# g-ch/DSP-map

Measured on AMD Instinct MI355X. Metric: map update() frames/sec @ 66x66x40, 24 particles/voxel; achieved HBM GB/s, higher is better.
Workload: dtype f32; 1 GPU; B: 66x66x40 @ 0.15 m, 24 particles/voxel, synthetic 640x480 depth @ 30 Hz (corridor scene, <=5000 points/frame after 0.1 m voxel filter), steady state after 300 frames; parallelism=1 GPU, n_points=3706, storage=runs of 64 voxel indices

## Files before the change

dsp-map_amd/csrc/dspmap_birth.h:

```cpp
#pragma once
#include "dspmap_device.h"

template <int NB>
__device__ __forceinline__ int block_excl_scan_multi(int (&v)[NB], int* s_tmp) {
    const int tid = threadIdx.x, w = tid >> 6, l = tid & 63, nw = blockDim.x >> 6;
    int inc[NB];
#pragma unroll
    for (int j = 0; j < NB; ++j) {
        inc[j] = wave_incl_scan_i(v[j]);
        if (l == 63) s_tmp[j * 16 + w] = inc[j];
    }
    __syncthreads();
    if (w == 0) {
        int run = 0;
#pragma unroll
        for (int j = 0; j < NB; ++j) {
            const int t = l < nw ? s_tmp[j * 16 + l] : 0;
            const int ti = wave_incl_scan_i(t);
            if (l < nw) s_tmp[j * 16 + l] = run + ti - t;
            run += __builtin_amdgcn_readlane(ti, 63);
        }
        if (l == 0) s_tmp[NB * 16] = run;
    }
    __syncthreads();
#pragma unroll
    for (int j = 0; j < NB; ++j) v[j] = inc[j] - v[j] + s_tmp[j * 16 + w];
    const int total = s_tmp[NB * 16];
    __syncthreads();
    return total;
}


#define BK 8
struct BirthView {
    const BirthSrc* stored;
    const float4* rot;
    const int* pyr;
    float cx, cy, cz;
    int n;
    bool live;
};
__device__ __forceinline__ BirthView birth_view(const DevState& s) {
    BirthView v;
    const FrameParams* fp = s.fpar;
    const int mode = fp->static_birth;
    v.live = mode == 1 && s.fs->view_epoch == fp->epoch;
    v.stored = fp->birth; v.rot = s.pt_rot; v.pyr = s.pt_pyr;
    v.cx = fp->cur_pos[0]; v.cy = fp->cur_pos[1]; v.cz = fp->cur_pos[2];
    v.n = mode == 1 ? (v.live ? fp->n_pts : s.fs->stale_n) : (mode == 2 ? s.fs->est_n : fp->n_birth);
    return v;
}
__device__ __forceinline__ BirthSrc birth_at(const BirthView& v, int i) {
    if (!v.live) return v.stored[i];
    const float4 r = v.rot[i];
    BirthSrc b;
    b.x = r.x + v.cx; b.y = r.y + v.cy; b.z = r.z + v.cz;
    b.nx = b.ny = b.nz = 0.f;
    b.intensity = v.pyr[i] >= 0 ? 0.f : -2.f;
    return b;
}
__device__ __forceinline__ bool birth_src_voxel(const MapDims& d, const DevState& s, const BirthSrc& src, float& cx, float& cy, float& cz, int& gv,
                                                const float* cp = nullptr) {
    if (!cp) cp = s.fs->cur_pos;
    cx = src.x - cp[0];
    cy = src.y - cp[1];
    cz = src.z - cp[2];
    if (!(src.intensity > -1.5f)) return false;
    if (voxel_of(d, cx, cy, cz, gv)) return true;
    gv = 0;
    return d.static_model != 0;
}

__device__ __forceinline__ void birth_rank_block(const MapDims& d, const DevState& s, const FilterParams& fp, bool fpar_pos = false) {
    const BirthView bv = birth_view(s);
    const float* cp = fpar_pos ? s.fpar->cur_pos : nullptr;
    const int n_birth = bv.n;
    __shared__ int s_tmp[BK * 16 + 1];
    const int tid = threadIdx.x, nt = blockDim.x;
    const int p_cur = s.fs->p_cur;
    const int nb = fp.nb_num;
    int run = 0;
    for (int base = 0; base < n_birth; base += nt * BK) {
        int v[BK];
        bool ok[BK];
#pragma unroll
        for (int j = 0; j < BK; ++j) {
            const int i = base + j * nt + tid;
            float cx, cy, cz; int gv;
            ok[j] = i < n_birth && birth_src_voxel(d, s, birth_at(bv, i), cx, cy, cz, gv, cp);
            v[j] = ok[j] ? 1 : 0;
            if (i < n_birth) s.plan_inside[i] = 0u;
        }
        const int tot = block_excl_scan_multi<BK>(v, s_tmp);
#pragma unroll
        for (int j = 0; j < BK; ++j)
            if (ok[j]) s.plan_pbase[base + j * nt + tid] = (int)(((long long)p_cur + 3ll * nb * (long long)(run + v[j])) % fp.tab_n);
        run += tot;
    }
    if (tid == 0) { s.fs->p_cur = (int)(((long long)p_cur + 3ll * nb * run) % fp.tab_n); s.fs->n_birth_ovf = 0; }
}

#define BIRTH_BUCKET_CAP 128
__device__ __forceinline__ void birth_child_thread(const MapDims& d, const DevState& s, const FilterParams& fp, float4* __restrict__ child,
                                                   int* __restrict__ vb_cnt, int* __restrict__ vb_idx, const int t, bool* inside_out = nullptr) {
    const BirthView bv = birth_view(s);
    const int n_birth = bv.n;
    const int nb = fp.nb_num;
    const int i = t / nb, k = t - i * nb;
    if (i >= n_birth) return;
    float cx, cy, cz; int gsrc;
    if (!birth_src_voxel(d, s, birth_at(bv, i), cx, cy, cz, gsrc)) return;
    const int c = (int)(((long long)s.plan_pbase[i] + 3 * k) % fp.tab_n);
    const float x = cx + s.p_tab[c];
    const float y = cy + s.p_tab[(c + 1) % fp.tab_n];
    const float z = cz + s.p_tab[(c + 2) % fp.tab_n];
    int gv = 0;
    int lv = -1;
    if (voxel_of_lv(d, x, y, z, gv, lv)) {
        if (inside_out) *inside_out = true; else atomicOr(&s.plan_inside[i], 1u << k);
        if (lv >= 0) {
            const int pos = atomicAdd(&vb_cnt[lv], 1);
            if (pos < BIRTH_BUCKET_CAP) vb_idx[(size_t)lv * BIRTH_BUCKET_CAP + pos] = t;
            else s.birth_ovf[atomicAdd(&s.fs->n_birth_ovf, 1)] = t;
        } else {
            lv = -1;
        }
    }
    child[t] = make_float4(x, y, z, __int_as_float(lv));
}
```

dsp-map_amd/csrc/dspmap_device.h:

```cpp
#pragma once
#include <hip/hip_runtime.h>
#include "dspmap_types.h"

#define WAVE 64

__device__ __forceinline__ int lane_id() { return (int)__lane_id(); }
__device__ __forceinline__ int sload_i(const int* p) {
    int v;
    asm volatile("s_load_dword %0, %1, 0x0\n\ts_waitcnt lgkmcnt(0)" : "=s"(v) : "s"(p));
    return v;
}
__device__ __forceinline__ void sload_i3(const int* p0, const int* p1, const int* p2, int& v0, int& v1, int& v2) {
    asm volatile("s_load_dword %0, %3, 0x0\n\ts_load_dword %1, %4, 0x0\n\ts_load_dword %2, %5, 0x0\n\ts_waitcnt lgkmcnt(0)"
                 : "=&s"(v0), "=&s"(v1), "=&s"(v2) : "s"(p0), "s"(p1), "s"(p2));
}
__device__ __forceinline__ void sload_i5(const int* p0, const int* p1, const int* p2, const int* p3, const int* p4, int& v0, int& v1, int& v2, int& v3, int& v4) {
    asm volatile("s_load_dword %0, %5, 0x0\n\ts_load_dword %1, %6, 0x0\n\ts_load_dword %2, %7, 0x0\n\ts_load_dword %3, %8, 0x0\n\ts_load_dword %4, %9, 0x0\n\ts_waitcnt lgkmcnt(0)"
                 : "=&s"(v0), "=&s"(v1), "=&s"(v2), "=&s"(v3), "=&s"(v4) : "s"(p0), "s"(p1), "s"(p2), "s"(p3), "s"(p4));
}
__device__ __forceinline__ void sload_i2(const int* p0, const int* p1, int& v0, int& v1) {
    asm volatile("s_load_dword %0, %2, 0x0\n\ts_load_dword %1, %3, 0x0\n\ts_waitcnt lgkmcnt(0)" : "=&s"(v0), "=&s"(v1) : "s"(p0), "s"(p1));
}
__device__ __forceinline__ void sload_i4(const int* p0, const int* p1, const int* p2, const int* p3, int& v0, int& v1, int& v2, int& v3) {
    asm volatile("s_load_dword %0, %4, 0x0\n\ts_load_dword %1, %5, 0x0\n\ts_load_dword %2, %6, 0x0\n\ts_load_dword %3, %7, 0x0\n\ts_waitcnt lgkmcnt(0)"
                 : "=&s"(v0), "=&s"(v1), "=&s"(v2), "=&s"(v3) : "s"(p0), "s"(p1), "s"(p2), "s"(p3));
}
__device__ __forceinline__ u64 lanemask_lt() { return (1ull << lane_id()) - 1ull; }

template <int CTRL, int ROW_MASK>
__device__ __forceinline__ float dpp_add_f(float v) {
    return v + __int_as_float(__builtin_amdgcn_update_dpp(0, __float_as_int(v), CTRL, ROW_MASK, 0xf, false));
}
template <int CTRL, int ROW_MASK>
__device__ __forceinline__ int dpp_add_i(int v) {
    return v + __builtin_amdgcn_update_dpp(0, v, CTRL, ROW_MASK, 0xf, false);
}
__device__ __forceinline__ float wave_incl_scan(float v) {
    v = dpp_add_f<0x111, 0xf>(v);
    v = dpp_add_f<0x112, 0xf>(v);
    v = dpp_add_f<0x114, 0xf>(v);
    v = dpp_add_f<0x118, 0xf>(v);
    v = dpp_add_f<0x142, 0xa>(v);
    v = dpp_add_f<0x143, 0xc>(v);
    return v;
}
__device__ __forceinline__ int wave_incl_scan_i(int v) {
    v = dpp_add_i<0x111, 0xf>(v);
    v = dpp_add_i<0x112, 0xf>(v);
    v = dpp_add_i<0x114, 0xf>(v);
    v = dpp_add_i<0x118, 0xf>(v);
    v = dpp_add_i<0x142, 0xa>(v);
    v = dpp_add_i<0x143, 0xc>(v);
    return v;
}
__device__ __forceinline__ float wave_sum(float v) {
    return __int_as_float(__builtin_amdgcn_readlane(__float_as_int(wave_incl_scan(v)), 63));
}
__device__ __forceinline__ float wave_sum_f(float v) {
#pragma unroll
    for (int o = 32; o > 0; o >>= 1) v += __shfl_xor(v, o, WAVE);
    return v;
}
__device__ __forceinline__ int wave_sum_i(int v) { return __builtin_amdgcn_readlane(wave_incl_scan_i(v), 63); }

__device__ __forceinline__ int wave_agg_inc(int* cnt, int key, bool active) {
    int pos = -1;
    u64 todo = __ballot(active);
    const int l = lane_id();
    while (todo) {
        const int leader = __ffsll((long long)todo) - 1;
        const int k = __shfl(key, leader, WAVE);
        const bool mine = active && key == k;
        const u64 grp = __ballot(mine);
        int base = 0;
        if (l == leader) base = atomicAdd(&cnt[k], (int)__popcll(grp));
        base = __shfl(base, leader, WAVE);
        if (mine) pos = base + (int)__popcll(grp & ((1ull << l) - 1ull));
        todo &= ~grp;
    }
    return pos;
}
__device__ __forceinline__ int wave_agg_inc1(int* cnt, bool active) {
    const u64 grp = __ballot(active);
    if (!grp) return -1;
    const int l = lane_id();
    const int leader = __ffsll((long long)grp) - 1;
    int base = 0;
    if (l == leader) base = atomicAdd(cnt, (int)__popcll(grp));
    base = __shfl(base, leader, WAVE);
    return active ? base + (int)__popcll(grp & ((1ull << l) - 1ull)) : -1;
}
__device__ __forceinline__ void wave_count_add(int* cnt, bool active) {
    const u64 grp = __ballot(active);
    if (grp && lane_id() == __ffsll((long long)grp) - 1) atomicAdd(cnt, (int)__popcll(grp));
}

__device__ __forceinline__ unsigned wave_or_u32(unsigned v) {
    v |= (unsigned)__builtin_amdgcn_update_dpp(0, (int)v, 0x111, 0xf, 0xf, false);
    v |= (unsigned)__builtin_amdgcn_update_dpp(0, (int)v, 0x112, 0xf, 0xf, false);
    v |= (unsigned)__builtin_amdgcn_update_dpp(0, (int)v, 0x114, 0xf, 0xf, false);
    v |= (unsigned)__builtin_amdgcn_update_dpp(0, (int)v, 0x118, 0xf, 0xf, false);
    v |= (unsigned)__builtin_amdgcn_update_dpp(0, (int)v, 0x142, 0xa, 0xf, false);
    v |= (unsigned)__builtin_amdgcn_update_dpp(0, (int)v, 0x143, 0xc, 0xf, false);
    return (unsigned)__builtin_amdgcn_readlane((int)v, 63);
}
__device__ __forceinline__ u64 wave_or_u64(u64 v) {
    return ((u64)wave_or_u32((unsigned)(v >> 32)) << 32) | (u64)wave_or_u32((unsigned)v);
}
__device__ __forceinline__ void quat_mul(const float a[4], const float b[4], float r[4]) {
    r[0] = a[0] * b[0] - a[1] * b[1] - a[2] * b[2] - a[3] * b[3];
    r[1] = a[0] * b[1] + a[1] * b[0] + a[2] * b[3] - a[3] * b[2];
    r[2] = a[0] * b[2] + a[2] * b[0] + a[3] * b[1] - a[1] * b[3];
    r[3] = a[0] * b[3] + a[3] * b[0] + a[1] * b[2] - a[2] * b[1];
}
__device__ __forceinline__ void rotate_by_quat(float vx, float vy, float vz, const float q[4], float out[3]) {
    float vq[4] = {0.f, vx, vy, vz};
    float n2 = q[1] * q[1] + q[2] * q[2] + q[3] * q[3] + q[0] * q[0];
    float inv[4] = {__fdiv_rn(q[0], n2), __fdiv_rn(-q[1], n2), __fdiv_rn(-q[2], n2), __fdiv_rn(-q[3], n2)};
    float t[4], r[4];
    quat_mul(q, vq, t);
    quat_mul(t, inv, r);
    out[0] = r[1]; out[1] = r[2]; out[2] = r[3];
}

__device__ __forceinline__ float dot3(float x, float y, float z, const float* n) {
    return x * n[0] + y * n[1] + z * n[2];
}

__device__ __forceinline__ int pyramid_of(const MapDims& d, const float* ph, const float* pv, float x, float y, float z) {
    if (!(dot3(x, y, z, ph) >= 0.f && dot3(x, y, z, ph + 3 * d.np_h) <= 0.f &&
          dot3(x, y, z, pv) <= 0.f && dot3(x, y, z, pv + 3 * d.np_v) >= 0.f))
        return -1;
    int lo = 0, hi = d.np_h - 1;
    while (lo < hi) {
        int mid = (lo + hi) >> 1;
        if (dot3(x, y, z, ph + 3 * (mid + 1)) <= 0.f) hi = mid; else lo = mid + 1;
    }
    const int h = lo;
    lo = 0; hi = d.np_v - 1;
    while (lo < hi) {
        int mid = (lo + hi) >> 1;
        if (dot3(x, y, z, pv + 3 * (mid + 1)) >= 0.f) hi = mid; else lo = mid + 1;
    }
    return h * d.np_v + lo;
}

__device__ __forceinline__ float div_res(const MapDims& d, float a) {
    if (d.div_ok) {
        const float q0 = a * d.rcp_res;
        const float r = __fmaf_rn(-q0, d.res, a);
        return __fmaf_rn(r, d.rcp_res, q0);
    }
    return __fdiv_rn(a, d.res);
}
__device__ __forceinline__ bool voxel_of(const MapDims& d, float px, float py, float pz, int& gidx) {
    if (fabsf(px) >= d.half_x || fabsf(py) >= d.half_y || fabsf(pz) >= d.half_z) return false;
    const int x = (int)div_res(d, px + d.half_x);
    const int y = (int)div_res(d, py + d.half_y);
    const int z = (int)div_res(d, pz + d.half_z);
    gidx = (int)(__umul24((unsigned)z, (unsigned)(d.ny * d.nx)) + __umul24((unsigned)y, (unsigned)d.nx) + (unsigned)x);
    return (unsigned)gidx < (unsigned)d.v_glob;
}

__device__ __forceinline__ int lv_of_xyz(const MapDims& d, int x, int y, int zl) {
    if (!d.tiling) return (int)(__umul24((unsigned)zl, (unsigned)(d.ny * d.nx)) + __umul24((unsigned)y, (unsigned)d.nx) + (unsigned)x);
    return ((((zl >> 2) * d.ncy + (y >> 2)) * d.ncx + (x >> 2)) << 6) | ((zl & 3) << 4) | ((y & 3) << 2) | (x & 3);
}
__device__ __forceinline__ int lv_of_true(const MapDims& d, int t) {
    if (!d.tiling) return t;
    const int zc = d.ny * d.nx;
    const int zl = t / zc, rest = t - zl * zc, y = rest / d.nx, x = rest - y * d.nx;
    return lv_of_xyz(d, x, y, zl);
}
__device__ __forceinline__ int lv_of_g(const MapDims& d, int gv) {
    const int t = gv - d.v_base;
    return (t >= 0 && t < d.v_true) ? lv_of_true(d, t) : -1;
}
__device__ __forceinline__ int g_of_lv(const MapDims& d, int lv) {
    if (!d.tiling) return lv + d.v_base;
    const int c = lv >> 6;
    const int cx = c % d.ncx, r = c / d.ncx, cy = r % d.ncy, cz = r / d.ncy;
    const int x = cx * 4 + (lv & 3), y = cy * 4 + ((lv >> 2) & 3), zl = cz * 4 + ((lv >> 4) & 3);
    if (x >= d.nx || y >= d.ny || zl >= d.z_hi - d.z_lo) return -1;
    return ((d.z_lo + zl) * d.ny + y) * d.nx + x;
}
__device__ __forceinline__ int tile_gbase(const MapDims& d, int BX) {
    if (!d.tiling) return d.v_base + BX * 64;
    const int cx = BX % d.ncx, r = BX / d.ncx, cy = r % d.ncy, cz = r / d.ncy;
    return ((d.z_lo + cz * 4) * d.ny + cy * 4) * d.nx + cx * 4;
}
__device__ __forceinline__ int lane_goff(const MapDims& d, int lane) {
    return d.tiling ? (((lane >> 4) & 3) * d.ny + ((lane >> 2) & 3)) * d.nx + (lane & 3) : lane;
}
__device__ __forceinline__ void cube_box(const MapDims& d, int BX, int& x0, int& y0, int& z0) {
    const int cx = BX % d.ncx, r = BX / d.ncx, cy = r % d.ncy, cz = r / d.ncy;
    x0 = cx * 4; y0 = cy * 4; z0 = d.z_lo + cz * 4;
}
__device__ __forceinline__ bool voxel_of_lv(const MapDims& d, float px, float py, float pz, int& gidx, int& lv) {
    if (fabsf(px) >= d.half_x || fabsf(py) >= d.half_y || fabsf(pz) >= d.half_z) return false;
    const int x = (int)div_res(d, px + d.half_x);
    const int y = (int)div_res(d, py + d.half_y);
    const int z = (int)div_res(d, pz + d.half_z);
    gidx = (int)(__umul24((unsigned)z, (unsigned)(d.ny * d.nx)) + __umul24((unsigned)y, (unsigned)d.nx) + (unsigned)x);
    if (!((unsigned)gidx < (unsigned)d.v_glob)) return false;
    const int zl = z - d.z_lo;
    lv = (unsigned)zl < (unsigned)(d.z_hi - d.z_lo) ? lv_of_xyz(d, x, y, zl) : -1;
    return true;
}

__device__ __forceinline__ float axis_u(float a, float mu, float sigma, float inv_sigma) {
    const float dlt = a - mu;
    const float q0 = dlt * inv_sigma;
    const float rr = __fmaf_rn(-q0, sigma, dlt);
    float z = __fmaf_rn(rr, inv_sigma, q0);
    z = __builtin_amdgcn_fmed3f(z, -9.9f, 9.9f);
    return floorf(z * 1000.f + 10000.f) - 10000.f;
}
__device__ __forceinline__ float pair_gk(float px, float py, float pz, float ox, float oy, float oz,
                                         float sigma, float inv_sigma, float c3) {
    const float ux = axis_u(px, ox, sigma, inv_sigma);
    const float uy = axis_u(py, oy, sigma, inv_sigma);
    const float uz = axis_u(pz, oz, sigma, inv_sigma);
    const float s = ux * ux + uy * uy + uz * uz;
    return c3 * __builtin_amdgcn_exp2f(s * -7.213475204444817e-07f);
}

typedef float f2v __attribute__((ext_vector_type(2)));
__device__ __forceinline__ f2v axis_u2(f2v a, f2v mu, float sigma, float inv_sigma) {
    const f2v dlt = a - mu;
    const f2v q0 = dlt * inv_sigma;
    const f2v rr = __builtin_elementwise_fma(-q0, (f2v)(sigma), dlt);
    f2v z = __builtin_elementwise_fma(rr, (f2v)(inv_sigma), q0);
    z.x = __builtin_amdgcn_fmed3f(z.x, -9.9f, 9.9f);
// ... 182 lines not shown
```

dsp-map_amd/csrc/dspmap_kernels.hip:

```cpp
#include <hip/hip_runtime.h>
#include "dspmap_device.h"
#include "dspmap_kernels.h"
#include "dspmap_birth.h"

#define RESET_PLANES 1
#define RESET_OBS 2
#define RESET_PRED 4

__global__ void k_reset(MapDims d, DevState s, int flags) {
    const float qw = s.fpar->quat[0], qx = s.fpar->quat[1], qy = s.fpar->quat[2], qz = s.fpar->quat[3];
    const float cx = s.fpar->cur_pos[0], cy = s.fpar->cur_pos[1], cz = s.fpar->cur_pos[2];
    const int gt = blockIdx.x * blockDim.x + threadIdx.x;
    const int gn = gridDim.x * blockDim.x;
    if (flags & RESET_PLANES) {
        const float q[4] = {qw, qx, qy, qz};
        const int nh = d.np_h + 1, nv = d.np_v + 1;
        for (int i = gt; i < nh + nv; i += gn) {
            float o[3];
            if (i < nh) {
                rotate_by_quat(s.planes_h0[3 * i], s.planes_h0[3 * i + 1], s.planes_h0[3 * i + 2], q, o);
                s.planes_h[3 * i] = o[0]; s.planes_h[3 * i + 1] = o[1]; s.planes_h[3 * i + 2] = o[2];
            } else {
                const int j = i - nh;
                rotate_by_quat(s.planes_v0[3 * j], s.planes_v0[3 * j + 1], s.planes_v0[3 * j + 2], q, o);
// ... 793 lines not shown
            const int wave = tid >> 6, l = tid & 63;
            const u64 cmask = (spl == 1 ? ~0ull : spl == 2 ? 0x5555555555555555ull : spl == 4 ? 0x1111111111111111ull : 0x0101010101010101ull) << sub;
            int run = 0, round = 0;
            for (int base = 0; base < O; base += WU_TPB, ++round) {
                const int o = base + tid;
                bool keep = false;
                float4 z = make_float4(0.f, 0.f, 0.f, 0.f);
                int oi = 0;
                if (o < O) {
                    int k = 0;
                    for (int q = 1; q < d.nbins; ++q) k += (o >= s_off[q]) ? 1 : 0;
                    oi = s_bin[k] * DSP_OBS_CAP + (o - s_off[k]);
                    z = s.obs[oi];
                    keep = z.w >= lo && z.w <= hi;
                }
                const u64 bal = __ballot(keep) & cmask;
                int* wc = s_wc + (round & 1) * 32;
                if (l < spl) wc[wave * 8 + l] = (int)__popcll(bal);
                __syncthreads();
                int off = run, tot = 0;
                for (int w = 0; w < WU_TPB / 64; ++w) { const int c = wc[w * 8 + sub]; tot += c; off += w < wave ? c : 0; }
                if (keep) {
                    const int pos = (off + (int)__popcll(bal & lanemask_lt())) * spl + sub;
                    s_len[pos] = z.w;
                    z.w = __fdiv_rn(fp.p_det, ck_from_fix(s.obs_ck[oi]) + add);
                    s_o[pos] = z;
                }
                run += tot;
            }
            n_mine = run;
        }
        __syncthreads();
        float sum = 0.f;
        if (valid && !occluded) {
            if (SKIP) {
                for (int j = 0; j < n_mine; ++j) {
                    const int o = j * spl + sub;
                    if (fabsf(s_len[o] - dist) > fp.cull_r) continue;
                    const float4 z = s_o[o];
                    sum += pair_gk(p.x, p.y, p.z, z.x, z.y, z.z, fp.sigma_ob, fp.inv_sigma_ob, fp.pdf_c3) * z.w;
                }
            } else {
                int o = sub;
                for (; o + spl < O; o += 2 * spl) {
                    const float4 z = s_o[o], z2 = s_o[o + spl];
                    const f2v gk = pair_gk2(f2v{p.x, p.x}, f2v{p.y, p.y}, f2v{p.z, p.z}, f2v{z.x, z2.x}, f2v{z.y, z2.y}, f2v{z.z, z2.z},
                                            fp.sigma_ob, fp.inv_sigma_ob, fp.pdf_c3);
                    if (fabsf(s_len[o] - dist) <= fp.cull_r) sum += gk.x * z.w;
                    if (fabsf(s_len[o + spl] - dist) <= fp.cull_r) sum += gk.y * z2.w;
                }
                if (o < O && fabsf(s_len[o] - dist) <= fp.cull_r) {
                    const float4 z = s_o[o];
                    sum += pair_gk(p.x, p.y, p.z, z.x, z.y, z.z, fp.sigma_ob, fp.inv_sigma_ob, fp.pdf_c3) * z.w;
                }
            }
        }
        if (spl >= 2) sum += __shfl_xor(sum, 1, WAVE);
        if (spl >= 4) sum += __shfl_xor(sum, 2, WAVE);
        if (spl >= 8) sum += __shfl_xor(sum, 4, WAVE);
        if (valid && !occluded && sub == 0) s.w[s.fov_slot_s[ri]] = p.w * ((1.f - fp.p_det) + sum);
    }
}

__device__ __forceinline__ void birth_split_wave(const MapDims& d, const DevState& s, const FilterParams& fp, int i, int2* cvr = nullptr,
                                                 const unsigned* inside_in = nullptr) {
    const BirthView bv = birth_view(s);
    if (cvr) *cvr = make_int2(0, 0);
    if (i >= bv.n) return;
    const int l = lane_id();
    const BirthSrc src = birth_at(bv, i);
    BirthPlan pl;
    pl.gvox = -1; pl.n_static = 0; pl.inside = 0; pl.pbase = pl.vbase = pl.rbase = 0;
    int gv;
    const bool ok = birth_src_voxel(d, s, src, pl.cx, pl.cy, pl.cz, gv);
    int n_static = 0;
    if (ok) {
        pl.gvox = gv;
        const int lv = lv_of_g(d, gv);
        if (lv >= 0) {
            float ws = 0.f, wsd = 0.f, wd = 0.f;
            for (int e = 0; e < d.mw; ++e) {
                const int sl = e * 64 + l;
                const u64 m = s.mask[(size_t)lv * d.mw + e] & ~s.nbmask[(size_t)lv * d.mw + e];
                if (sl < d.slots && ((m >> l) & 1ull)) {
                    const size_t idx = pidx(d, lv, sl);
                    const V2 pv = ld_vel(s, idx);
                    const float vabs = fabsf(pv.x) + fabsf(pv.y) + 0.f;
                    const float w = s.w[idx];
                    if (vabs < 0.1f) ws += w; else if (vabs < 0.5f) wsd += w; else wd += w;
                }
            }
            ws = wave_sum(ws); wsd = wave_sum(wsd); wd = wave_sum(wd);
            const float total = ws + wd + wsd;
            const float m_s = __fdiv_rn(ws, total), m_d = __fdiv_rn(wd, total), m_sd = __fdiv_rn(wsd, total);
            const float p_s = (m_s + m_s + m_sd) * 0.5f;
            const float p_d = (m_d + m_d + m_sd) * 0.5f;
            const float p_s_n = __fdiv_rn(p_s, p_s + p_d);
            const float f = (float)fp.model_nb * p_s_n;
            int ns = (f != f) ? 0 : (int)f;
            n_static = max(fp.min_static_nb, ns);
        }
    }
    pl.n_static = n_static;
    if (l == 0) { s.plan[i] = pl; s.nstatic[i] = n_static; }
    if (cvr && ok && src.intensity > 0.01f) {
        const unsigned inside = inside_in ? *inside_in : s.plan_inside[i];
        const int nb = fp.nb_num;
        const int model_end = src.nx > -100.f ? fp.model_nb : n_static;
        auto below = [](int k) { return k >= 32 ? ~0u : ((1u << k) - 1u); };
        const int lo = min(n_static, nb), mid = min(max(model_end, lo), nb);
        *cvr = make_int2(3 * __popc(inside & below(mid) & ~below(lo)), 3 * __popc(inside & below(nb) & ~below(mid)));
    }
}
__global__ void k_birth_split(MapDims d, DevState s, FilterParams fp) {
    birth_split_wave(d, s, fp, (int)(blockIdx.x * (blockDim.x / WAVE) + threadIdx.x / WAVE));
}

__device__ __forceinline__ void birth_point_wave(const MapDims& d, const DevState& s, const FilterParams& fp, int i, float4* __restrict__ child,
                                                 int* __restrict__ vb_cnt, int* __restrict__ vb_idx, int2* cvr) {
    const BirthView bv = birth_view(s);
    *cvr = make_int2(0, 0);
    if (i >= bv.n) return;
    const int l = lane_id(), nb = fp.nb_num;
    const BirthSrc src = birth_at(bv, i);
    const int pb = s.plan_pbase[i];
    BirthPlan pl;
    pl.gvox = -1; pl.n_static = 0; pl.inside = 0; pl.pbase = pl.vbase = pl.rbase = 0;
    int gv;
    const bool ok = birth_src_voxel(d, s, src, pl.cx, pl.cy, pl.cz, gv);
    if (!ok) {
        if (l == 0) { s.plan[i] = pl; s.nstatic[i] = 0; s.plan_inside[i] = 0u; }
        return;
    }
    pl.gvox = gv;
    const int lvs = lv_of_g(d, gv);
    const bool own = lvs >= 0;
    const int lvq = own ? lvs : 0;
    const int c = (int)(((long long)pb + 3 * min(l, nb - 1)) % fp.tab_n);
    const float t0 = s.p_tab[c], t1 = s.p_tab[(c + 1) % fp.tab_n], t2 = s.p_tab[(c + 2) % fp.tab_n];
    u64 mwd[2] = {0ull, 0ull};
    for (int e = 0; e < d.mw; ++e) mwd[e] = s.mask[(size_t)lvq * d.mw + e] & ~s.nbmask[(size_t)lvq * d.mw + e];
    V2 pv[2];
    float pw[2];
    bool on[2];
#pragma unroll
    for (int e = 0; e < 2; ++e) {
        const int sl = e * 64 + l;
        on[e] = own && e < d.mw && sl < d.slots && ((mwd[e] >> l) & 1ull);
        const size_t idx = pidx(d, lvq, on[e] ? sl : 0);
        pv[e] = ld_vel(s, idx);
        pw[e] = s.w[idx];
    }
    bool in = false;
    if (l < nb) {
        const int t = i * nb + l;
        const float x = pl.cx + t0, y = pl.cy + t1, z = pl.cz + t2;
        int gvc = 0, lvc = -1;
        if (voxel_of_lv(d, x, y, z, gvc, lvc)) {
            in = true;
            if (lvc >= 0) {
                const int pos = atomicAdd(&vb_cnt[lvc], 1);
                if (pos < BIRTH_BUCKET_CAP) vb_idx[(size_t)lvc * BIRTH_BUCKET_CAP + pos] = t;
                else s.birth_ovf[atomicAdd(&s.fs->n_birth_ovf, 1)] = t;
            } else {
                lvc = -1;
            }
        }
        child[t] = make_float4(x, y, z, __int_as_float(lvc));
    }
    const unsigned inside = (unsigned)__ballot(in);
    int n_static = 0;
    if (own) {
        float ws = 0.f, wsd = 0.f, wd = 0.f;
#pragma unroll
        for (int e = 0; e < 2; ++e) {
            if (on[e]) {
                const float vabs = fabsf(pv[e].x) + fabsf(pv[e].y) + 0.f;
                if (vabs < 0.1f) ws += pw[e]; else if (vabs < 0.5f) wsd += pw[e]; else wd += pw[e];
            }
        }
        ws = wave_sum(ws); wsd = wave_sum(wsd); wd = wave_sum(wd);
        const float total = ws + wd + wsd;
        const float m_s = __fdiv_rn(ws, total), m_d = __fdiv_rn(wd, total), m_sd = __fdiv_rn(wsd, total);
        const float p_s = (m_s + m_s + m_sd) * 0.5f;
        const float p_d = (m_d + m_d + m_sd) * 0.5f;
        const float p_s_n = __fdiv_rn(p_s, p_s + p_d);
        const float f = (float)fp.model_nb * p_s_n;
        const int ns = (f != f) ? 0 : (int)f;
        n_static = max(fp.min_static_nb, ns);
    }
    pl.n_static = n_static;
    if (l == 0) { s.plan[i] = pl; s.nstatic[i] = n_static; s.plan_inside[i] = inside; }
    if (src.intensity > 0.01f) {
        const int model_end = src.nx > -100.f ? fp.model_nb : n_static;
        auto below = [](int k) { return k >= 32 ? ~0u : ((1u << k) - 1u); };
        const int lo = min(n_static, nb), mid = min(max(model_end, lo), nb);
        *cvr = make_int2(3 * __popc(inside & below(mid) & ~below(lo)), 3 * __popc(inside & below(nb) & ~below(mid)));
    }
}

__device__ __forceinline__ void ck_sum_block(const MapDims& d, const DevState& s, const FilterParams& fp, float* s_red) {
    const int tid = threadIdx.x;
    float acc = 0.f;
    if (tid < 512) {
        for (int i = tid; i < d.np; i += 512) acc += s.part_inv[i];
        s_red[tid] = acc;
    }
    __syncthreads();
    for (int o = 256; o > 0; o >>= 1) {
        if (tid < o) s_red[tid] += s_red[tid + o];
        __syncthreads();
    }
    if (tid == 0) {
        s.fs->expected_newborn = frame_lambda(s, fp);
        s.fs->newborn_w = fp.nb_weight * s_red[0];
    }
}
__global__ void __launch_bounds__(1024) k_birth_rank(MapDims d, DevState s, FilterParams fp, int with_ck_sum) {
    __shared__ float s_red[512];
    if (with_ck_sum) ck_sum_block(d, s, fp, s_red);
    birth_rank_block(d, s, fp);
}
__global__ void __launch_bounds__(1024) k_birth_split_rank(MapDims d, DevState s, FilterParams fp, int with_ck_sum) {
    if (blockIdx.x == gridDim.x - 1) {
        __shared__ float s_red[512];
        if (with_ck_sum) ck_sum_block(d, s, fp, s_red);
        birth_rank_block(d, s, fp);
    } else birth_split_wave(d, s, fp, (int)(blockIdx.x * (1024 / WAVE) + threadIdx.x / WAVE));
}


__global__ void k_birth_children(MapDims d, DevState s, FilterParams fp, float4* __restrict__ child,
                                 int* __restrict__ vb_cnt, int* __restrict__ vb_idx) {
    birth_child_thread(d, s, fp, child, vb_cnt, vb_idx, (int)(blockIdx.x * blockDim.x + threadIdx.x));
}

__global__ void __launch_bounds__(1024) k_birth_cursors(MapDims d, DevState s, FilterParams fp) {
    const BirthView bv = birth_view(s);
    const int n_birth = bv.n;
    __shared__ int s_tmp[BK * 16 + 1];
    const int tid = threadIdx.x;
    const int v_cur = s.fs->v_cur, r_cur = s.fs->r_cur;
    const int nb = fp.nb_num;
    int run_v = 0, run_r = 0;
    for (int base = 0; base < n_birth; base += 1024 * BK) {
        int gvox[BK], nst[BK];
        unsigned inside[BK];
        float inten[BK], snx[BK];
#pragma unroll
        for (int j = 0; j < BK; ++j) {
            const int i = base + j * 1024 + tid;
            gvox[j] = -1; nst[j] = 0; inside[j] = 0u; inten[j] = 0.f; snx[j] = 0.f;
            if (i < n_birth) {
                gvox[j] = s.plan[i].gvox; inside[j] = s.plan_inside[i];
                nst[j] = s.nstatic[i];
                const BirthSrc b = birth_at(bv, i);
                inten[j] = b.intensity; snx[j] = b.nx;
            }
        }
        int cv[BK], cr[BK];
#pragma unroll
        for (int j = 0; j < BK; ++j) {
            cv[j] = 0; cr[j] = 0;
            if (gvox[j] >= 0 && inten[j] > 0.01f) {
                const int model_end = snx[j] > -100.f ? fp.model_nb : nst[j];
                for (int k = nst[j]; k < nb; ++k) {
                    if (!((inside[j] >> k) & 1u)) continue;
                    if (k < model_end) cv[j] += 3; else cr[j] += 3;
                }
            }
        }
        const int totv = block_excl_scan_multi<BK>(cv, s_tmp);
        const int totr = block_excl_scan_multi<BK>(cr, s_tmp);
#pragma unroll
        for (int j = 0; j < BK; ++j) {
            if (gvox[j] >= 0) {
                BirthPlan* pl = &s.plan[base + j * 1024 + tid];
                pl->n_static = nst[j];
                pl->vbase = (int)(((long long)v_cur + run_v + cv[j]) % fp.tab_n);
                pl->rbase = (int)(((long long)r_cur + run_r + cr[j]) % max(fp.rtab_n, 1));
            }
        }
        run_v += totv; run_r += totr;
    }
    if (tid == 0) {
        s.fs->v_cur = (int)(((long long)v_cur + run_v) % fp.tab_n);
        s.fs->r_cur = (int)(((long long)r_cur + run_r) % max(fp.rtab_n, 1));
    }
}

__device__ __forceinline__ float rand_float(const DevState& s, const FilterParams& fp, int c, float lo, float hi) {
    const int r = s.r_tab[c % max(fp.rtab_n, 1)];
    return lo + __fdiv_rn((float)r, __fdiv_rn((float)2147483647, (hi - lo)));
}

template <bool FUSED>
__global__ void __launch_bounds__(256) k_birth_insert(MapDims d, DevState s, FilterParams fp, const float4* __restrict__ child,
                               const int* __restrict__ vb_cnt, const int* __restrict__ vb_idx, int* __restrict__ part_birth,
                               const u64* __restrict__ nbsnap, int wg_off) {
    if (s.xq && s.fpar->from_ring && __hip_atomic_load(s.xq + 8, __ATOMIC_RELAXED, __HIP_MEMORY_SCOPE_AGENT) == (int)(s.fpar->ring_pos + 1u)) {
        if (threadIdx.x < 2) part_birth[blockIdx.x * 2 + threadIdx.x] = 0;
        return;
    }
    const BirthView bv = birth_view(s);
    const int n_birth = bv.n;
    const int t = blockIdx.x * blockDim.x + threadIdx.x;
    const int nb = fp.nb_num;
    const int i = t / nb, k = t - i * nb;
    bool born = false, dropped = false;
    int f_vbase = 0, f_rbase = 0;
    if (FUSED) {
        __shared__ int s_part[4][4];
        const int tid = (int)threadIdx.x;
        const int i_first = (int)((blockIdx.x * blockDim.x) / (unsigned)nb);
        const int G = min(i_first, n_birth) >> 4;
        const int ngr = (n_birth + 15) >> 4;
        int acc[4] = {0, 0, 0, 0};
        for (int g = tid; g < ngr; g += 256) {
            const int2 w = s.birth_cvr[wg_off + g];
            acc[2] += w.x; acc[3] += w.y;
            if (g < G) { acc[0] += w.x; acc[1] += w.y; }
        }
        int2 loc = make_int2(0, 0);
        for (int j = G << 4; j < min(i, n_birth); ++j) { const int2 c = s.birth_cvr[j]; loc.x += c.x; loc.y += c.y; }
#pragma unroll
        for (int q = 0; q < 4; ++q) { acc[q] = wave_sum_i(acc[q]); if (lane_id() == 0) s_part[tid >> 6][q] = acc[q]; }
        __syncthreads();
#pragma unroll
        for (int q = 0; q < 4; ++q) acc[q] = (s_part[0][q] + s_part[1][q]) + (s_part[2][q] + s_part[3][q]);
        const int v0 = s.fs->v_cur_in, r0 = s.fs->r_cur_in;
        f_vbase = (int)(((long long)v0 + acc[0] + loc.x) % fp.tab_n);
        f_rbase = (int)(((long long)r0 + acc[1] + loc.y) % max(fp.rtab_n, 1));
        if (t == 0) {
            s.fs->v_cur = (int)(((long long)v0 + acc[2]) % fp.tab_n);
            s.fs->r_cur = (int)(((long long)r0 + acc[3]) % max(fp.rtab_n, 1));
        }
    }
    if (bv.live && t == 0) s.fs->stale_n = n_birth;
    if (i < n_birth) {
        const BirthPlan pl = s.plan[i];
        const unsigned pl_inside = s.plan_inside[i];
        const float4 ch = child[t];
        const BirthSrc src = birth_at(bv, i);
        if (bv.live && k == 0) const_cast<BirthSrc*>(bv.stored)[i] = src;
        const float newborn_w = s.fs->newborn_w;
        if (pl.gvox >= 0 && ((pl_inside >> k) & 1u)) {
            const int lv = __float_as_int(ch.w);
            if (lv >= 0) {
                const int n = min(vb_cnt[lv], BIRTH_BUCKET_CAP);
                u64 occ[2];
                for (int e = 0; e < d.mw; ++e) occ[e] = s.mask[(size_t)lv * d.mw + e] | (nbsnap ? nbsnap[(size_t)lv * d.mw + e] : 0ull);
                float vx = 0.f, vy = 0.f;
                if (k >= pl.n_static && src.intensity > 0.01f) {
                    const int model_end = src.nx > -100.f ? fp.model_nb : pl.n_static;
                    const unsigned lo_mask = (k >= 32 ? ~0u : ((1u << k) - 1u)) & ~((pl.n_static >= 32) ? ~0u : ((1u << pl.n_static) - 1u));
                    const unsigned before = pl_inside & lo_mask;
                    if (k < model_end) {
                        const int rank = __popc(before);
                        const int cv = (int)(((long long)(FUSED ? f_vbase : pl.vbase) + 3 * rank) % fp.tab_n);
                        vx = src.nx + 4 * s.v_tab[cv];
                        vy = src.ny + 4 * s.v_tab[(cv + 1) % fp.tab_n];
                    } else {
                        const unsigned model_bits = (model_end >= 32) ? ~0u : ((1u << model_end) - 1u);
                        const int rank = __popc(before & ~model_bits);
                        const int cr = (FUSED ? f_rbase : pl.rbase) + 3 * rank;
                        vx = rand_float(s, fp, cr, -1.5f, 1.5f);
                        vy = rand_float(s, fp, cr + 1, -1.5f, 1.5f);
                    }
                }
                int rank = 0;
                const int n_all = vb_cnt[lv];
                bool recorded = n_all > BIRTH_BUCKET_CAP;
                const int4* bl4 = reinterpret_cast<const int4*>(vb_idx + (size_t)lv * BIRTH_BUCKET_CAP);
                for (int j = 0; j < n; j += 16) {
                    int4 v4[4];
#pragma unroll
                    for (int u = 0; u < 4; ++u) v4[u] = bl4[(j >> 2) + u];
#pragma unroll
                    for (int u = 0; u < 4; ++u) {
                        const int o[4] = {v4[u].x, v4[u].y, v4[u].z, v4[u].w};
#pragma unroll
                        for (int q = 0; q < 4; ++q) {
                            const bool valid = j + u * 4 + q < n;
                            rank += (valid && o[q] < t) ? 1 : 0;
                            recorded |= valid && (o[q] == t);
                        }
                    }
                }
                if (n_all > BIRTH_BUCKET_CAP) {
                    const int n_ovf = s.fs->n_birth_ovf;
                    for (int j = 0; j < n_ovf; ++j) {
                        const int o = s.birth_ovf[j];
                        rank += (o < t && __float_as_int(child[o].w) == lv) ? 1 : 0;
                    }
                }
                int sl = -1;
                if (recorded) {
                    int r = rank;
                    for (int e = 0; e < d.mw && sl < 0; ++e) {
                        const int nbits = min(64, d.slots - e * 64);
                        const u64 valid = nbits >= 64 ? ~0ull : ((1ull << nbits) - 1ull);
                        u64 fr = ~occ[e] & valid;
                        const int nf = (int)__popcll(fr);
                        if (r >= nf) { r -= nf; continue; }
                        for (int q = 0; q < r; ++q) fr &= fr - 1ull;
                        sl = e * 64 + (__ffsll((long long)fr) - 1);
                    }
                }
                if (sl >= 0) {
                    const size_t idx = pidx(d, lv, sl);
                    st_pos(s, idx, ch.x, ch.y, ch.z);
                    st_vel(s, idx, vx, vy);
                    note_speed(s, vx, vy);
                    if (vx != 0.f || vy != 0.f) s.tile_moving[lv >> 6] = 1;
                    s.w[idx] = newborn_w;
                    atomicOr(&s.nbmask[(size_t)lv * d.mw + (sl >> 6)], 1ull << (sl & 63));
                    s.tile_live[lv >> 6] = 1;
                    if (s.vis_bits) {
                        const int tl = lv >> 6;
                        if (!((__hip_atomic_load(&s.vis_bits[tl >> 5], __ATOMIC_RELAXED, __HIP_MEMORY_SCOPE_AGENT) >> (tl & 31)) & 1u)) atomicOr(&s.vis_bits[tl >> 5], 1u << (tl & 31));
                    }
                    born = true;
                } else {
                    dropped = true;
                }
            }
        }
    }
    __shared__ int s_bc[2];
    if (threadIdx.x < 2) s_bc[threadIdx.x] = 0;
    __syncthreads();
    const u64 bb = __ballot(born), bd = __ballot(dropped);
    if (lane_id() == 0) {
        if (bb) atomicAdd(&s_bc[0], (int)__popcll(bb));
        if (bd) atomicAdd(&s_bc[1], (int)__popcll(bd));
    }
    __syncthreads();
    if (threadIdx.x < 2) part_birth[blockIdx.x * 2 + threadIdx.x] = s_bc[threadIdx.x];
}

__global__ void __launch_bounds__(256) k_occ_count(MapDims d, DevState s, float thr) {
    __shared__ int s_c[4];
    const int tv = blockIdx.x * 256 + threadIdx.x;
    const bool occ = tv < d.v_true && s.res4[lv_of_true(d, tv)].x > thr;
    const u64 b = __ballot(occ);
    if (lane_id() == 0) s_c[threadIdx.x >> 6] = (int)__popcll(b);
    __syncthreads();
    if (threadIdx.x == 0) s.blk_cnt[blockIdx.x] = s_c[0] + s_c[1] + s_c[2] + s_c[3];
}
__global__ void __launch_bounds__(1024) k_occ_scan(DevState s, int nblk) {
    __shared__ int s_tmp[17];
    __shared__ int s_run;
    if (threadIdx.x == 0) s_run = 0;
    __syncthreads();
    for (int base = 0; base < nblk; base += 1024) {
        const int i = base + threadIdx.x;
        const int v = i < nblk ? s.blk_cnt[i] : 0;
        int tot;
        const int ex = block_excl_scan_1024(v, s_tmp, &tot);
        if (i < nblk) s.blk_cnt[i] = s_run + ex;
        __syncthreads();
        if (threadIdx.x == 0) s_run += tot;
        __syncthreads();
    }
    if (threadIdx.x == 0) s.fs->occupied_count = s_run;
}
__global__ void __launch_bounds__(256) k_occ_emit(MapDims d, DevState s, float thr, int cap) {
    __shared__ int s_c[4];
    const int tv = blockIdx.x * 256 + threadIdx.x;
    const bool occ = tv < d.v_true && s.res4[lv_of_true(d, tv)].x > thr;
    const u64 b = __ballot(occ);
    const int w = threadIdx.x >> 6;
    if (lane_id() == 0) s_c[w] = (int)__popcll(b);
    __syncthreads();
    int off = s.blk_cnt[blockIdx.x];
    for (int k = 0; k < w; ++k) off += s_c[k];
    if (occ) {
        const int pos = off + (int)__popcll(b & lanemask_lt());
        if (pos < cap) {
            const int index = tv + d.v_base;
            const int zc = d.ny * d.nx;
            const int zi = index / zc;
            const int rest = index - zi * zc;
            const int yi = rest / d.nx;
            const int xi = rest - yi * d.nx;
            const float cx = -d.half_x + d.res * 0.5f, cy = -d.half_y + d.res * 0.5f, cz = -d.half_z + d.res * 0.5f;
            s.occ_xyz[3 * pos] = (float)xi * d.res + cx;
            s.occ_xyz[3 * pos + 1] = (float)yi * d.res + cy;
            s.occ_xyz[3 * pos + 2] = (float)zi * d.res + cz;
        }
    }
}



void launch_frame_setup(const LaunchCtx& c, bool reset_obs) {
    const int flags = RESET_PLANES | RESET_PRED | (reset_obs ? RESET_OBS : 0);
    const int n = c.d.np * DSP_OBS_CAP;
// ... 230 lines not shown
```

Before: 6467 frames/s.

## Aggregate birth bucket atomics per wave and hoist birth-insert loads ahead of ring check

Replaces per-thread atomicAdd on voxel bucket counters with a wave-aggregated single atomic per distinct key, used in both child-generation paths. In k_birth_insert, all global loads (plan, child, source, cvr prefix words, cursors) are issued up front before the ring-skip check so their latency overlaps. The serial per-thread loop that summed the local prefix of birth_cvr becomes a shared-memory wave scan. This adds register pressure and a loop over distinct keys per wave, and makes early-exit blocks issue loads they would have skipped.

```diff
diff --git a/dsp-map_amd/csrc/dspmap_birth.h b/dsp-map_amd/csrc/dspmap_birth.h
--- a/dsp-map_amd/csrc/dspmap_birth.h
+++ b/dsp-map_amd/csrc/dspmap_birth.h
@@ -43,11 +43,12 @@
 __device__ __forceinline__ BirthView birth_view(const DevState& s) {
     BirthView v;
     const FrameParams* fp = s.fpar;
-    const int mode = fp->static_birth;
-    v.live = mode == 1 && s.fs->view_epoch == fp->epoch;
+    const int mode = fp->static_birth, epoch = fp->epoch, n_pts = fp->n_pts, n_given = fp->n_birth;
+    const int view_epoch = s.fs->view_epoch, stale_n = s.fs->stale_n, est_n = s.fs->est_n;
+    v.live = mode == 1 && view_epoch == epoch;
     v.stored = fp->birth; v.rot = s.pt_rot; v.pyr = s.pt_pyr;
     v.cx = fp->cur_pos[0]; v.cy = fp->cur_pos[1]; v.cz = fp->cur_pos[2];
-    v.n = mode == 1 ? (v.live ? fp->n_pts : s.fs->stale_n) : (mode == 2 ? s.fs->est_n : fp->n_birth);
+    v.n = mode == 1 ? (v.live ? n_pts : stale_n) : (mode == 2 ? est_n : n_given);
     return v;
 }
 __device__ __forceinline__ BirthSrc birth_at(const BirthView& v, int i) {
@@ -101,30 +102,34 @@
 }
 
 #define BIRTH_BUCKET_CAP 128
+__device__ __forceinline__ void birth_bucket_put(const DevState& s, int* __restrict__ vb_cnt, int* __restrict__ vb_idx, const int lv, const int t) {
+    const int pos = wave_agg_inc_once(vb_cnt, lv, lv >= 0);
+    if (lv >= 0) {
+        if (pos < BIRTH_BUCKET_CAP) vb_idx[(size_t)lv * BIRTH_BUCKET_CAP + pos] = t;
+        else s.birth_ovf[atomicAdd(&s.fs->n_birth_ovf, 1)] = t;
+    }
+}
 __device__ __forceinline__ void birth_child_thread(const MapDims& d, const DevState& s, const FilterParams& fp, float4* __restrict__ child,
                                                    int* __restrict__ vb_cnt, int* __restrict__ vb_idx, const int t, bool* inside_out = nullptr) {
     const BirthView bv = birth_view(s);
     const int n_birth = bv.n;
     const int nb = fp.nb_num;
     const int i = t / nb, k = t - i * nb;
-    if (i >= n_birth) return;
     float cx, cy, cz; int gsrc;
-    if (!birth_src_voxel(d, s, birth_at(bv, i), cx, cy, cz, gsrc)) return;
-    const int c = (int)(((long long)s.plan_pbase[i] + 3 * k) % fp.tab_n);
-    const float x = cx + s.p_tab[c];
-    const float y = cy + s.p_tab[(c + 1) % fp.tab_n];
-    const float z = cz + s.p_tab[(c + 2) % fp.tab_n];
-    int gv = 0;
     int lv = -1;
-    if (voxel_of_lv(d, x, y, z, gv, lv)) {
-        if (inside_out) *inside_out = true; else atomicOr(&s.plan_inside[i], 1u << k);
-        if (lv >= 0) {
-            const int pos = atomicAdd(&vb_cnt[lv], 1);
-            if (pos < BIRTH_BUCKET_CAP) vb_idx[(size_t)lv * BIRTH_BUCKET_CAP + pos] = t;
-            else s.birth_ovf[atomicAdd(&s.fs->n_birth_ovf, 1)] = t;
+    if (i < n_birth && birth_src_voxel(d, s, birth_at(bv, i), cx, cy, cz, gsrc)) {
+        const int c = (int)(((long long)s.plan_pbase[i] + 3 * k) % fp.tab_n);
+        const float x = cx + s.p_tab[c];
+        const float y = cy + s.p_tab[(c + 1) % fp.tab_n];
+        const float z = cz + s.p_tab[(c + 2) % fp.tab_n];
+        int gv = 0;
+        if (voxel_of_lv(d, x, y, z, gv, lv)) {
+            if (inside_out) *inside_out = true; else atomicOr(&s.plan_inside[i], 1u << k);
+            if (lv < 0) lv = -1;
         } else {
             lv = -1;
         }
+        child[t] = make_float4(x, y, z, __int_as_float(lv));
     }
-    child[t] = make_float4(x, y, z, __int_as_float(lv));
+    birth_bucket_put(s, vb_cnt, vb_idx, lv, t);
 }
diff --git a/dsp-map_amd/csrc/dspmap_device.h b/dsp-map_amd/csrc/dspmap_device.h
--- a/dsp-map_amd/csrc/dspmap_device.h
+++ b/dsp-map_amd/csrc/dspmap_device.h
@@ -79,6 +79,23 @@
         todo &= ~grp;
     }
     return pos;
+}
+__device__ __forceinline__ int wave_agg_inc_once(int* cnt, int key, bool active) {
+    const int l = lane_id();
+    u64 todo = __ballot(active);
+    int gsize = 0, grank = 0, lead = l;
+    while (todo) {
+        const int first = __ffsll((long long)todo) - 1;
+        const int k = __builtin_amdgcn_readlane(key, first);
+        const bool mine = active && key == k;
+        const u64 grp = __ballot(mine);
+        if (mine) { gsize = (int)__popcll(grp); grank = (int)__popcll(grp & ((1ull << l) - 1ull)); lead = first; }
+        todo &= ~grp;
+    }
+    int base = 0;
+    if (active && lead == l) base = atomicAdd(&cnt[key], gsize);
+    base = __shfl(base, lead, WAVE);
+    return active ? base + grank : -1;
 }
 __device__ __forceinline__ int wave_agg_inc1(int* cnt, bool active) {
     const u64 grp = __ballot(active);
diff --git a/dsp-map_amd/csrc/dspmap_kernels.hip b/dsp-map_amd/csrc/dspmap_kernels.hip
--- a/dsp-map_amd/csrc/dspmap_kernels.hip
+++ b/dsp-map_amd/csrc/dspmap_kernels.hip
@@ -969,22 +969,16 @@
         pw[e] = s.w[idx];
     }
     bool in = false;
+    const int t = i * nb + l;
+    int lvc = -1;
     if (l < nb) {
-        const int t = i * nb + l;
         const float x = pl.cx + t0, y = pl.cy + t1, z = pl.cz + t2;
-        int gvc = 0, lvc = -1;
-        if (voxel_of_lv(d, x, y, z, gvc, lvc)) {
-            in = true;
-            if (lvc >= 0) {
-                const int pos = atomicAdd(&vb_cnt[lvc], 1);
-                if (pos < BIRTH_BUCKET_CAP) vb_idx[(size_t)lvc * BIRTH_BUCKET_CAP + pos] = t;
-                else s.birth_ovf[atomicAdd(&s.fs->n_birth_ovf, 1)] = t;
-            } else {
-                lvc = -1;
-            }
-        }
+        int gvc = 0;
+        if (voxel_of_lv(d, x, y, z, gvc, lvc)) in = true;
+        if (!in || lvc < 0) lvc = -1;
         child[t] = make_float4(x, y, z, __int_as_float(lvc));
     }
+    birth_bucket_put(s, vb_cnt, vb_idx, lvc, t);
     const unsigned inside = (unsigned)__ballot(in);
     int n_static = 0;
     if (own) {
@@ -1115,37 +1109,84 @@
 __global__ void __launch_bounds__(256) k_birth_insert(MapDims d, DevState s, FilterParams fp, const float4* __restrict__ child,
                                const int* __restrict__ vb_cnt, const int* __restrict__ vb_idx, int* __restrict__ part_birth,
                                const u64* __restrict__ nbsnap, int wg_off) {
-    if (s.xq && s.fpar->from_ring && __hip_atomic_load(s.xq + 8, __ATOMIC_RELAXED, __HIP_MEMORY_SCOPE_AGENT) == (int)(s.fpar->ring_pos + 1u)) {
-        if (threadIdx.x < 2) part_birth[blockIdx.x * 2 + threadIdx.x] = 0;
-        return;
-    }
+    const int from_ring = s.fpar->from_ring;
+    const unsigned ring_pos = s.fpar->ring_pos;
+    const bool ring = s.xq && from_ring;
+    const int xq_pos = (int)(ring_pos + 1u);
     const BirthView bv = birth_view(s);
     const int n_birth = bv.n;
+    int xq_word = 0;
+    if (ring) xq_word = __hip_atomic_load(s.xq + 8, __ATOMIC_RELAXED, __HIP_MEMORY_SCOPE_AGENT);
+    const int tid = (int)threadIdx.x;
     const int t = blockIdx.x * blockDim.x + threadIdx.x;
     const int nb = fp.nb_num;
     const int i = t / nb, k = t - i * nb;
+    const int i_first = (int)((blockIdx.x * blockDim.x) / (unsigned)nb), i_last = (int)((blockIdx.x * blockDim.x + 255u) / (unsigned)nb);
+    const int G = min(i_first, n_birth) >> 4;
+    const int w_end = min(i_last + 1, n_birth);
+    const int ngr = (n_birth + 15) >> 4;
+    int2 we = make_int2(0, 0), wr = make_int2(0, 0);
+    int2 wg0 = make_int2(0, 0);
+    int v0 = 0, r0 = 0;
+    if (FUSED) {
+        if ((G << 4) + tid < w_end) we = s.birth_cvr[(G << 4) + tid];
+        if (tid < 16 && (G << 4) + 256 + tid < w_end) wr = s.birth_cvr[(G << 4) + 256 + tid];
+        if (tid < ngr) wg0 = s.birth_cvr[wg_off + tid];
+        v0 = s.fs->v_cur_in; r0 = s.fs->r_cur_in;
+    }
+    BirthPlan pl;
+    pl.gvox = -1; pl.n_static = 0;
+    unsigned pl_inside = 0u;
+    float4 ch = make_float4(0.f, 0.f, 0.f, 0.f);
+    BirthSrc src;
+    src.nx = src.ny = 0.f; src.intensity = 0.f;
+    float newborn_w = 0.f;
+    if (i < n_birth) {
+        pl = s.plan[i];
+        pl_inside = s.plan_inside[i];
+        ch = child[t];
+        src = birth_at(bv, i);
+        newborn_w = s.fs->newborn_w;
+    }
+    int acc[4] = {0, 0, 0, 0};
+    if (FUSED) {
+        acc[2] = wg0.x; acc[3] = wg0.y;
+        if (tid < G) { acc[0] = wg0.x; acc[1] = wg0.y; }
+        for (int g = tid + 256; g < ngr; g += 256) {
+            const int2 w = s.birth_cvr[wg_off + g];
+            acc[2] += w.x; acc[3] += w.y;
+            if (g < G) { acc[0] += w.x; acc[1] += w.y; }
+        }
+    }
+    asm volatile("" : "+v"(xq_word));
+    if (ring && xq_word == xq_pos) {
+        if (threadIdx.x < 2) part_birth[blockIdx.x * 2 + threadIdx.x] = 0;
+        return;
+    }
     bool born = false, dropped = false;
     int f_vbase = 0, f_rbase = 0;
     if (FUSED) {
         __shared__ int s_part[4][4];
-        const int tid = (int)threadIdx.x;
-        const int i_first = (int)((blockIdx.x * blockDim.x) / (unsigned)nb);
-        const int G = min(i_first, n_birth) >> 4;
-        const int ngr = (n_birth + 15) >> 4;
-        int acc[4] = {0, 0, 0, 0};
-        for (int g = tid; g < ngr; g += 256) {
-            const int2 w = s.birth_cvr[wg_off + g];
-            acc[2] += w.x; acc[3] += w.y;
-            if (g < G) { acc[0] += w.x; acc[1] += w.y; }
-        }
-        int2 loc = make_int2(0, 0);
-        for (int j = G << 4; j < min(i, n_birth); ++j) { const int2 c = s.birth_cvr[j]; loc.x += c.x; loc.y += c.y; }
-#pragma unroll
-        for (int q = 0; q < 4; ++q) { acc[q] = wave_sum_i(acc[q]); if (lane_id() == 0) s_part[tid >> 6][q] = acc[q]; }
+        __shared__ int2 s_pre[256 + 16];
+        __shared__ int2 s_run[4];
+        const int wv = tid >> 6;
+#pragma unroll
+        for (int q = 0; q < 4; ++q) { acc[q] = wave_sum_i(acc[q]); if (lane_id() == 0) s_part[wv][q] = acc[q]; }
+        const int2 inc = make_int2(wave_incl_scan_i(we.x), wave_incl_scan_i(we.y));
+        s_pre[tid] = make_int2(inc.x - we.x, inc.y - we.y);
+        if (lane_id() == 63) s_run[wv] = inc;
+        if (wv == 0) {
+            const int2 rinc = make_int2(wave_incl_scan_i(wr.x), wave_incl_scan_i(wr.y));
+            if (tid < 16) s_pre[256 + tid] = make_int2(rinc.x - wr.x, rinc.y - wr.y);
+        }
         __syncthreads();
 #pragma unroll
         for (int q = 0; q < 4; ++q) acc[q] = (s_part[0][q] + s_part[1][q]) + (s_part[2][q] + s_part[3][q]);
-        const int v0 = s.fs->v_cur_in, r0 = s.fs->r_cur_in;
+        const int idx = min(i, n_birth) - (G << 4);
+        int2 loc = s_pre[idx];
+#pragma unroll
+        for (int q = 0; q < 4; ++q)
+            if (q < (idx >> 6)) { loc.x += s_run[q].x; loc.y += s_run[q].y; }
         f_vbase = (int)(((long long)v0 + acc[0] + loc.x) % fp.tab_n);
         f_rbase = (int)(((long long)r0 + acc[1] + loc.y) % max(fp.rtab_n, 1));
         if (t == 0) {
@@ -1155,12 +1196,7 @@
     }
     if (bv.live && t == 0) s.fs->stale_n = n_birth;
     if (i < n_birth) {
-        const BirthPlan pl = s.plan[i];
-        const unsigned pl_inside = s.plan_inside[i];
-        const float4 ch = child[t];
-        const BirthSrc src = birth_at(bv, i);
         if (bv.live && k == 0) const_cast<BirthSrc*>(bv.stored)[i] = src;
-        const float newborn_w = s.fs->newborn_w;
         if (pl.gvox >= 0 && ((pl_inside >> k) & 1u)) {
             const int lv = __float_as_int(ch.w);
             if (lv >= 0) {
```

Result: faster. 6632 frames/s (median of 6 runs) (+2.5%).
